# fnothaft/spark-bam

Hardware: AMD Instinct MI355X
Metric: compressed BAM GB/s for compute-splits + full-check (whole node, 1/2/4/8 GPU) (higher is better)
Workload: dtype u8

## Files before the change

spark-bam_amd/csrc/sbam_inflate.hip:

```cpp
#include <type_traits>

#include "sbam_internal.h"

namespace sbam {

#define SB_DEV __device__ __forceinline__

enum : int32_t { INF_OK = 0, INF_SHORT = 1, INF_DATA = 2, INF_OVERFLOW = 3 };

constexpr uint32_t kTokPad = 0x7fffu;
constexpr uint32_t kTokDist = 0x8000u;

SB_DEV uint64_t tok_region(int64_t uoff, int64_t b) {
  return (((uint64_t)uoff + 15) & ~15ull) + 32ull * (uint64_t)b;
}
SB_DEV int32_t tok_region_cap(int32_t us) { return (us + 16) / 2; }
SB_DEV uint64_t tok_arena_need(int32_t us) { return ((uint64_t)(2 * us + 32) + 15) & ~15ull; }

constexpr int kDecThreads = 256;
constexpr int kRows = 80;
constexpr int kLitSorted = 0;
constexpr int kClTab = 0;
constexpr int kLensLitRow = 32;
constexpr int kLensDistRow = 68;
constexpr int kDistSorted = 288;
constexpr int kEpoch = 4;
constexpr int kParkMin = 16;

constexpr uint8_t kClOrder[19] = {16, 17, 18, 0, 8, 7, 9, 6, 10, 5, 11, 4, 12, 3, 13, 2, 14, 1, 15};

struct Slice {
  uint8_t *base;
  SB_DEV uint8_t *b(int i) const { return base + (i >> 2) * (kDecThreads * 4) + (i & 3); }
  SB_DEV uint32_t *w(int row) const { return reinterpret_cast<uint32_t *>(base + row * (kDecThreads * 4)); }
};

template <int B, int E, class F>
SB_DEV void sfor(F &&f) {
  if constexpr (B < E) {
    f(std::integral_constant<int, B>{});
    sfor<B + 1, E>(f);
  }
}

struct Canon {
  uint32_t lim[16];
  int32_t pk[16];
};

SB_DEV int canon_decode(const Canon &c, uint64_t bb, int &len, bool &valid, int &hist) {
  const uint32_t rev = __builtin_bitreverse32((uint32_t)bb) >> 17;
  int32_t p = c.pk[1];
  sfor<1, 15>([&](auto I) {
    constexpr int l = decltype(I)::value;
    p = rev >= c.lim[l] ? c.pk[l + 1] : p;
  });
  const int L = p & 31;
  valid = rev < c.lim[15];
  len = valid ? L : 1;
  hist = (p >> 5) & 511;
  return valid ? (int)(rev >> (15 - L)) + (p >> 14) : 0;
}

SB_DEV int canon_decode_sel(const Canon &a, const Canon &b, bool useB, uint64_t bb, int &len, bool &valid,
                            int &hist) {
  const uint32_t rev = __builtin_bitreverse32((uint32_t)bb) >> 17;
  int32_t p = useB ? b.pk[1] : a.pk[1];
  sfor<1, 15>([&](auto I) {
    constexpr int l = decltype(I)::value;
    const uint32_t lim = useB ? b.lim[l] : a.lim[l];
    const int32_t pn = useB ? b.pk[l + 1] : a.pk[l + 1];
    p = rev >= lim ? pn : p;
  });
  const int L = p & 31;
  valid = rev < (useB ? b.lim[15] : a.lim[15]);
  len = valid ? L : 1;
  hist = (p >> 5) & 511;
  return valid ? (int)(rev >> (15 - L)) + (p >> 14) : 0;
}

struct Cnt15 {
  uint64_t a = 0, b = 0, c = 0;
  SB_DEV void add(uint32_t l, uint64_t v) {
    const uint32_t w = (l >= 7) + (l >= 14);
    const uint64_t inc = v << (9 * (l - 7 * w));
    a += w == 0 ? inc : 0ull;
    b += w == 1 ? inc : 0ull;
    c += w == 2 ? inc : 0ull;
  }
  SB_DEV uint32_t get(uint32_t l) const {
    const uint32_t w = (l >= 7) + (l >= 14);
    const uint64_t x = w == 0 ? a : w == 1 ? b : c;
    return (uint32_t)(x >> (9 * (l - 7 * w))) & 511u;
  }
};

template <int NW>
SB_DEV int canon_build(const uint32_t (&lens)[NW], const Slice &sl, int sorted_off, bool lit, Canon &c) {
  Cnt15 cnt, lo;
#pragma unroll
  for (int dw = 0; dw < NW; dw++) {
    const uint32_t w = lens[dw];
#pragma unroll 1
    for (int j = 0; j < 8; j++) {
      const uint32_t v = (w >> (4 * j)) & 15u;
      if (v) {
        cnt.add(v, 1);
        if (lit && dw * 8 + j < 256) lo.add(v, 1);
      }
    }
  }
  int left = 1, maxl = 0;
  bool over = false;
  uint32_t code = 0;
  int32_t offs = 0;
  Cnt15 cur;
  sfor<1, 16>([&](auto I) {
    constexpr int l = decltype(I)::value;
    const uint32_t k = cnt.get(l);
    left = 2 * left - (int)k;
    over |= left < 0;
    maxl = k ? l : maxl;
    c.lim[l] = (code + k) << (15 - l);
    const int32_t bse = offs - (int32_t)code;
    const uint32_t hist = (uint32_t)offs + (lit ? lo.get(l) : 0u);
    c.pk[l] = (int32_t)(((uint32_t)bse << 14) | (hist << 5) | (uint32_t)l);
    cur.add(l, (uint64_t)offs);
    offs += (int32_t)k;
    code = (code + k) << 1;
  });
  c.lim[0] = 0;
  c.pk[0] = 0;
  if (over || (left > 0 && maxl > 1)) return -1;
#pragma unroll
  for (int dw = 0; dw < NW; dw++) {
    const uint32_t w = lens[dw];
#pragma unroll 1
    for (int j = 0; j < 8; j++) {
      const uint32_t v = (w >> (4 * j)) & 15u;
      if (v) {
        const uint32_t pos = cur.get(v);
        cur.add(v, 1);
        *sl.b(sorted_off + (int)pos) = (uint8_t)(dw * 8 + j);
      }
    }
  }
  return 0;
}

SB_DEV uint32_t csel(uint64_t m, uint32_t a, uint32_t b) {
  uint32_t r;
  asm("v_cndmask_b32 %0, %1, %2, %3" : "=v"(r) : "v"(a), "v"(b), "s"(m));
  return r;
}
SB_DEV uint32_t sel16(const uint32_t (&A)[16], uint32_t i) {
  const uint64_t m0 = __builtin_amdgcn_ballot_w64((i & 1u) != 0), m1 = __builtin_amdgcn_ballot_w64((i & 2u) != 0),
                 m2 = __builtin_amdgcn_ballot_w64((i & 4u) != 0), m3 = __builtin_amdgcn_ballot_w64((i & 8u) != 0);
  uint32_t t[8], u[4];
#pragma unroll
  for (int k = 0; k < 8; k++) t[k] = csel(m0, A[2 * k], A[2 * k + 1]);
#pragma unroll
  for (int k = 0; k < 4; k++) u[k] = csel(m1, t[2 * k], t[2 * k + 1]);
  return csel(m3, csel(m2, u[0], u[1]), csel(m2, u[2], u[3]));
}

struct TokOut {
  uint32_t t0, t1, t2, t3;
  uint32_t p0, p1, p2, p3;
  int n;
  bool pend;
  uint64_t cur;
};

SB_DEV bool tok_store(TokOut &to, uint32_t a, uint32_t b, uint32_t c, uint32_t d, uint8_t *pool) {
  *reinterpret_cast<uint4 *>(pool + to.cur) = make_uint4(a, b, c, d);
  to.cur += 16;
  return true;
}

SB_DEV bool tok_put(TokOut &to, uint32_t t, uint8_t *pool) {
  to.t0 = __builtin_amdgcn_alignbit(to.t1, to.t0, 16);
  to.t1 = __builtin_amdgcn_alignbit(to.t2, to.t1, 16);
  to.t2 = __builtin_amdgcn_alignbit(to.t3, to.t2, 16);
  to.t3 = __builtin_amdgcn_alignbit(t, to.t3, 16);
  if (++to.n < 8) return true;
  bool ok = true;
  if (to.pend) ok = tok_store(to, to.p0, to.p1, to.p2, to.p3, pool);
  to.p0 = to.t0;
  to.p1 = to.t1;
  to.p2 = to.t2;
  to.p3 = to.t3;
  to.pend = true;
  to.n = 0;
  return ok;
}

enum : int { S_NEXT = 0, S_HDR = 1, S_HUFF = 2, S_STORED = 3, S_DONE = 4, S_EXIT = 5, S_PARK = 6 };


struct Bits {
  uint64_t bb;
  int bc;
  int left;
  uint32_t rp, nx;
  SB_DEV uint32_t peek(int n) const { return (uint32_t)bb & ((1u << n) - 1u); }
  SB_DEV void drop(int n) {
    bb >>= n;
    bc -= n;
    left -= n;
  }
  SB_DEV void refill_hbm(const uint32_t *src) {
    if (bc <= 32) {
      bb |= (uint64_t)src[rp] << bc;
      bc += 32;
      rp++;
    }
  }
};

__global__ __launch_bounds__(kDecThreads, 2) void k_inflate_slow(const uint8_t *__restrict__ d, int64_t D,
                                                                 BlockTable bt, TokPool tp,
                                                                 const int32_t *__restrict__ slow,
                                                                 const unsigned int *nslow,
                                                                 int32_t *__restrict__ status,
                                                                 int32_t *__restrict__ found,
                                                                 unsigned int *next_block) {
  __shared__ __attribute__((aligned(16))) uint8_t s_dec[kRows * kDecThreads * 4];
  const Slice sl{s_dec + 4 * threadIdx.x};
  const uint32_t *d32 = reinterpret_cast<const uint32_t *>(d);
  uint8_t *pool = tp.arena;

  int state = S_NEXT;
  int64_t blk = -1;
  const uint32_t *src = d32;
  uint32_t ldw = 0;
  Bits br{0, 0, 0, 0, 0};
  uint32_t A[16], B[8];
  uint32_t ws = 0;
#pragma unroll
  for (int k = 0; k < 16; k++) A[k] = 0;
#pragma unroll
  for (int k = 0; k < 8; k++) B[k] = 0;
  TokOut to{0, 0, 0, 0, 0, 0, 0, 0, 0, false, 0};
  Canon lc, dc;
  int32_t o = 0, us = 0, err = INF_OK, sleft = 0, fin = 0;
  bool drain = false;
  auto refill = [&]() {
    if (br.bc <= 32) {
      br.bb |= (uint64_t)br.nx << br.bc;
      br.bc += 32;
      br.rp++;
      br.nx = sel16(A, br.rp - ws);
    }
  };

  for (int it = 0;; it++) {
    if (state == S_NEXT) {
      const uint32_t i = atomicAdd(next_block, 1u);
      if (i >= *nslow) {
        state = S_EXIT;
      } else {
        blk = slow[i];
        const int64_t st = bt.start[blk];
        const int32_t hs = bt.hsize[blk], cs = bt.csize[blk];
        us = bt.usize[blk];
        o = 0;
        fin = 0;
        err = INF_OK;
        drain = false;
        const int32_t dlen = cs - hs - 8;
        if (us == 0) {
          state = S_DONE;
        } else if (us < 0 || us > 65536 || dlen < 0 || st + hs + dlen > D) {
          err = INF_DATA;
          state = S_DONE;
        } else {
          const uint64_t need = tok_arena_need(us);
          const uint64_t at = atomicAdd(tp.arena_used, (unsigned long long)need);
          if ((int64_t)(at + need) > tp.arena_cap) {
            err = INF_OVERFLOW;
            state = S_DONE;
          } else {
            tp.base[blk] = (int64_t)at;
            to.cur = at;
            to.n = 0;
            to.pend = false;
            const int64_t a = st + hs;
            src = d32 + (a >> 2);
            ldw = (uint32_t)(((a & 3) + dlen + 8 + 3) >> 2);
            const int skip = (int)(a & 3) * 8;
            br.bb = (uint64_t)src[0] >> skip;
            br.bc = 32 - skip;
            br.rp = 1;
            br.left = 8 * dlen;
            state = S_PARK;
          }
        }
      }
    }
    if ((it & (kEpoch - 1)) == 0) {
      if (__all(state == S_EXIT)) break;
      const uint64_t pk = __ballot(state == S_PARK);
      const uint64_t dc = __ballot(state == S_HUFF || state == S_STORED);
      if (pk && (__popcll(pk) >= kParkMin || dc == 0) && state == S_PARK) state = S_HDR;
    }
// ... 967 lines not shown
          tokA += cnt ? 1u : 0u;
          bytA += (cl ? lenv : 0u) + ((cnt && kind == K_LIT) ? 1u : 0u);
          pl = cl ? lenv : pl;
          st4 = live ? (cl ? 4u : 0u) : st4;
        };
        sfor<0, kCp>([&](auto J) {
          constexpr int jj = decltype(J)::value;
          const bool live = go && rp < seg_end;
          cp[jj] = (live && st4 == 0) ? (uint32_t)rp : ~0u;
          cc[jj] = tokA | (bytA << 12);
          if (__ballot(live) != 0) {
            if constexpr (jj * kCpSteps < kTR) {
              sfor<0, kCpSteps>([&](auto K) {
                constexpr int sj = jj * kCpSteps + decltype(K)::value;
                step(std::integral_constant<int, (sj < kTR ? sj : -1)>{});
              });
            } else {
#pragma unroll 2
              for (int k = 0; k < kCpSteps; k++) step(std::integral_constant<int, -1>{});
            }
          }
          if constexpr ((jj + 1) * kCpSteps == kTR) {
            stR = ((uint32_t)rp << 10) | (st4 << 7) | pl;
            bytR = bytA;
          }
        });
        while (__ballot(go && rp < seg_end) != 0) step(std::integral_constant<int, -1>{});
        exitEnd = ((uint32_t)rp << 10) | (st4 << 7) | pl;
      }
      WMARK(3);
      const SegResult own = nst > 0 ? SegResult{s1c & 4095u, s1c >> 12, s1e & ~1023u, (int)(s1e & 3u), false}
                                    : SegResult{tokA, bytA, exitEnd, ST_NONE, false};
      SegResult res = own;
      uint32_t nxt = lane == 0 ? own.exit : exitEnd;
      uint32_t bst = lane == 0 ? S : entry;
      bool ver = lane == 0;
      enum : int { kModeA = 0, kModeR = 1, kModeF = 2 };
      int mode = kModeA;
      uint32_t rjP = 0, rjs = 0, rjtk = 0;
      int f = 64;
      for (;;) {
        uint32_t pex = __shfl_up(nxt, 1);
        if (lane == 0) pex = S;
        bool upd = false;
        if (!ver && pex == bst) {
          ver = true;
          upd = nxt != own.exit;
          nxt = own.exit;
          res = own;
          mode = kModeA;
        }
        const uint64_t vs = __ballot(ver && res.stop != ST_NONE);
        f = uni(vs ? __ffsll((unsigned long long)vs) - 1 : 64);
        const bool need = lane > 0 && lane <= f && pex != bst;
        if (__ballot(need || upd) == 0) break;
        WADD(7, 1);
        if (need) {
          uint32_t st4 = (pex >> 7) & 4u;
          uint32_t pl = pex & 511u, tk = 0, by = 0;
          int rp = (int)(pex >> 10);
          auto next_cp = [&](uint32_t p) {
            uint32_t m = ~0u;
            sfor<0, kCp>([&](auto I) {
              const uint32_t x = cp[decltype(I)::value];
              m = (x >= p && x < m) ? x : m;
            });
            return m;
          };
          uint32_t tcp = next_cp((uint32_t)rp);
          mode = kModeF;
          for (;;) {
            if (st4 == 0 && (uint32_t)rp == tcp) {
              uint32_t cj = 0, sj = 0;
              sfor<0, kCp>([&](auto I) {
                const bool hit = cp[decltype(I)::value] == tcp;
                cj = hit ? cc[decltype(I)::value] : cj;
                sj = hit ? (uint32_t)(decltype(I)::value * kCpSteps) : sj;
              });
              const uint32_t P = tcp;
              mode = kModeR;
              rjP = P;
              rjs = sj;
              rjtk = tk;
              const bool h1 = nst >= 1 && s1p >= P, h2 = !h1 && nst >= 2 && s2p >= P;
              if (h1 || h2) {
                const uint32_t se = h1 ? s1e : s2e, sc = h1 ? s1c : s2c;
                res = SegResult{tk + (sc & 4095u) - (cj & 4095u), by + (sc >> 12) - (cj >> 12), se & ~1023u,
                                (int)(se & 3u), false};
                break;
              }
              if (nst <= 2) {
                res = SegResult{tk + tokA - (cj & 4095u), by + bytA - (cj >> 12), exitEnd, ST_NONE, false};
                break;
              }
              tcp = ~0u;
              mode = kModeF;
            }
            if (rp >= seg_end) {
              res = SegResult{tk, by, ((uint32_t)rp << 10) | (st4 << 7) | pl, ST_NONE, false};
              break;
            }
            uint32_t v;
            const uint32_t kind = wsym(wp, L, rp, st4, v);
            const bool outp = rp > pend;
            if (kind == K_SPEC || outp) {
              res = SegResult{tk, by, (uint32_t)rp << 10, outp ? ST_OUT : v == 0 ? ST_EOB : ST_ERR, false};
              break;
            }
            tk++;
            by += kind == K_LIT ? 1u : kind == K_LEN ? v - 253u : 0u;
            pl = kind == K_LEN ? v - 253u : pl;
            st4 = kind == K_LEN ? 4u : 0u;
            if ((uint32_t)rp > tcp) tcp = next_cp((uint32_t)rp);
          }
          nxt = res.stop != ST_NONE ? res.exit : res.exit;
          ver = true;
          bst = pex;
        }
      }
      WMARK(4);
      const bool act = lane <= f;
#ifdef SBAM_WAVE_STATS
      {
        const bool viaB = act && mode != kModeA;
        WADD(23, __ballot(act && mode == kModeF) != 0 ? 1 : 0);
        WADD(14, __popcll(__ballot(act)));
        WADD(15, __popcll(__ballot(viaB)));
        WADD(16, __popcll(__ballot(act && res.tok > 64)));
        WADD(17, __popcll(__ballot(act && res.tok > 96)));
        WADD(18, __popcll(__ballot(act && res.tok > 128)));
        WADD(19, __ballot(viaB) != 0 ? 1 : 0);
        WADD(20, __ballot(act && res.tok > 96) != 0 ? 1 : 0);
        WADD(21, __ballot(act && res.tok > 64) != 0 ? 1 : 0);
        WADD(22, __ballot(act && own.stop != ST_NONE) != 0 ? 1 : 0);
      }
#endif
      const uint32_t my_tok = act ? res.tok : 0u, my_byt = act ? res.byt : 0u;
      const uint32_t itok = wave_incl_scan(my_tok), ibyt = wave_incl_scan(my_byt);
      const uint32_t tot_tok = uni((uint32_t)__shfl(itok, 63)), tot_byt = uni((uint32_t)__shfl(ibyt, 63));
      const int stop_f = f < 64 ? uni(__shfl(res.stop, f)) : ST_NONE;
      if (stop_f == ST_ERR || stop_f == ST_OUT || out + (int)tot_byt > us || __ballot(act && res.bad) != 0) {
        ok = false;
        break;
      }
      if (ntok + (int)tot_tok > tcap) {
        const uint64_t need = tok_arena_need(us);
        uint64_t at = 0;
        if (lane == 0) at = atomicAdd(tp.arena_used, (unsigned long long)need);
        at = ((uint64_t)uni((uint32_t)__shfl((int)(at >> 32), 0)) << 32) | uni((uint32_t)__shfl((int)(uint32_t)at, 0));
        if ((int64_t)(at + need) > tp.arena_cap) {
          ok = false;
          break;
        }
        uint8_t *nreg = tp.arena + at;
        __builtin_amdgcn_fence(__ATOMIC_SEQ_CST, "workgroup");
        const int nb = 2 * ntok, nb16 = nb & ~15;
        for (int i = 16 * lane; i < nb16; i += 1024)
          *reinterpret_cast<uint4 *>(nreg + i) = *reinterpret_cast<const uint4 *>(reg + i);
        if (lane < (nb - nb16) / 2)
          reinterpret_cast<uint16_t *>(nreg + nb16)[lane] = reinterpret_cast<const uint16_t *>(reg + nb16)[lane];
        if (lane == 0) tp.base[b] = (int64_t)at;
        reg = nreg;
        tcap = 1 << 30;
      }
      bool tail = false;
      uint32_t tail_ti = 0, tail_st = 0;
      uint32_t r_lo = 0, r_hi = 0, r_tb = 0;
      if (act) {
        uint32_t start = __shfl_up(nxt, 1);
        if (lane == 0) start = S;
        uint32_t ti = (uint32_t)ntok + (itok - my_tok);
        auto run = [&](uint32_t st, int endp) {
          uint32_t st4 = (st >> 7) & 4u;
          int rp = (int)(st >> 10);
          while (rp < endp) {
            uint32_t v;
            const uint32_t kind = wsym(wp, L, rp, st4, v);
            if (kind == K_SPEC) break;
            st4 = kind == K_LEN ? 4u : 0u;
            *reinterpret_cast<uint16_t *>(reg + 2 * ti) = (uint16_t)v;
            ti++;
          }
        };
        WMARK(24);
        run(start, mode == kModeF ? seg_end : mode == kModeR ? (int)rjP : 0);
        WMARK(25);
        const uint32_t lo = mode == kModeR ? rjs : 0u;
        const uint32_t n = mode == kModeA ? res.tok : mode == kModeR ? res.tok - rjtk : 0u;
        const uint32_t hi = mode == kModeF ? 0u : min(lo + n, (uint32_t)kTR);
        const uint32_t tb = ti - lo;
        r_lo = lo;
        r_hi = hi;
        r_tb = tb;
        static_assert(kTR == 80, "one asm operand per register token dword");
        asm volatile("" : "+v"(tr[0]), "+v"(tr[1]), "+v"(tr[2]), "+v"(tr[3]), "+v"(tr[4]), "+v"(tr[5]), "+v"(tr[6]), "+v"(tr[7]), "+v"(tr[8]), "+v"(tr[9]), "+v"(tr[10]), "+v"(tr[11]), "+v"(tr[12]), "+v"(tr[13]), "+v"(tr[14]), "+v"(tr[15]), "+v"(tr[16]), "+v"(tr[17]), "+v"(tr[18]), "+v"(tr[19]), "+v"(tr[20]), "+v"(tr[21]), "+v"(tr[22]), "+v"(tr[23]), "+v"(tr[24]), "+v"(tr[25]), "+v"(tr[26]), "+v"(tr[27]), "+v"(tr[28]), "+v"(tr[29]), "+v"(tr[30]), "+v"(tr[31]), "+v"(tr[32]), "+v"(tr[33]), "+v"(tr[34]), "+v"(tr[35]), "+v"(tr[36]), "+v"(tr[37]), "+v"(tr[38]), "+v"(tr[39]));
        {
          const uint32_t par = tb & 1u;
          uint8_t *pa = reg + 2 * ((int64_t)ti - (int64_t)lo);
          if (par && lo == 0 && hi > 0) *reinterpret_cast<uint16_t *>(pa) = (uint16_t)tr[0];
          u32x4a *pv = reinterpret_cast<u32x4a *>(pa + 2 * par);
          uint32_t *pw = reinterpret_cast<uint32_t *>(pa + 2 * par);
          auto dw = [&](auto Q) {
            constexpr int q = decltype(Q)::value;
            const uint32_t nx = q + 1 < kTR / 2 ? tr[q + 1 < kTR / 2 ? q + 1 : q] : 0u;
            return par ? __builtin_amdgcn_alignbit(nx, tr[q], 16) : tr[q];
          };
          sfor<0, kTR / 8>([&](auto C) {
            constexpr int c = decltype(C)::value;
            const uint32_t a0 = dw(std::integral_constant<int, 4 * c>{}), a1 = dw(std::integral_constant<int, 4 * c + 1>{});
            const uint32_t a2 = dw(std::integral_constant<int, 4 * c + 2>{}), a3 = dw(std::integral_constant<int, 4 * c + 3>{});
            const uint32_t t0 = par + 8 * c;
            if (t0 >= lo && t0 + 8 <= hi) {
              pv[c] = u32x4a{a0, a1, a2, a3};
            } else if (t0 + 8 > lo && t0 < hi) {
              const uint32_t a[4] = {a0, a1, a2, a3};
#pragma unroll
              for (int k = 0; k < 4; k++) {
                const uint32_t u0 = t0 + 2 * k;
                const bool in0 = u0 >= lo && u0 < hi, in1 = u0 + 1 >= lo && u0 + 1 < hi;
                uint16_t *ph = reinterpret_cast<uint16_t *>(pw + 4 * c + k);
                if (in0 && in1) pw[4 * c + k] = a[k];
                else if (in0) ph[0] = (uint16_t)a[k];
                else if (in1) ph[1] = (uint16_t)(a[k] >> 16);
              }
            }
          });
        }
        WMARK(26);
        WMARK(27);
        tail = mode != kModeF && lo + n > (uint32_t)kTR;
        tail_st = lo <= (uint32_t)kTR ? stR : rjP << 10;
        tail_ti = lo <= (uint32_t)kTR ? tb + kTR : ti;
      }
      if (tail) {
        uint32_t st4 = (tail_st >> 7) & 4u, ti = tail_ti;
        int rp = (int)(tail_st >> 10);
        while (rp < seg_end) {
          uint32_t v;
          const uint32_t kind = wsym(wp, L, rp, st4, v);
          if (kind == K_SPEC) break;
          st4 = kind == K_LEN ? 4u : 0u;
          *reinterpret_cast<uint16_t *>(reg + 2 * ti) = (uint16_t)v;
          ti++;
        }
      }
      (void)r_lo;
      (void)r_hi;
      (void)r_tb;
      WMARK(28);
      out += (int)tot_byt;
      ntok += (int)tot_tok;
      if (f < 64) {
        pos = (int)(uni((uint32_t)__shfl(res.exit, f)) >> 10);
        break;
      }
      S = uni((uint32_t)__shfl(nxt, 63));
    }
  }
  if (ok && out != us) ok = false;
#ifdef SBAM_WAVE_STATS
  ws_[8] = __builtin_amdgcn_s_memtime() - wt0_;
  if (lane == 0)
    for (int i = 0; i < 29; i++) atomicAdd(&g_wave_stats[i], (unsigned long long)ws_[i]);
#endif
  if (lane == 0) {
    if (ok) {
      status[b] = INF_OK;
      found[b] = us;
    } else if (stored) {
      slow[bt.n + atomicAdd(nslow + 3, 1u)] = (int32_t)b;
    } else {
      slow[atomicAdd(nslow, 1u)] = (int32_t)b;
    }
  }
}

__global__ __launch_bounds__(64) void k_inflate_stored(const uint8_t *__restrict__ d, BlockTable bt, TokPool tp,
                                                      uint8_t *__restrict__ out, int32_t *__restrict__ status,
                                                      int32_t *__restrict__ found, int32_t *__restrict__ slow,
                                                      unsigned int *nslow) {
  __shared__ uint32_t seg[2 * kMaxStored];
  const unsigned n = nslow[3];
  for (unsigned i = blockIdx.x; i < n; i += gridDim.x) {
    const int64_t b = slow[bt.n + i];
    const int64_t a = bt.start[b] + bt.hsize[b], U0 = bt.uoff[b];
    const int32_t dlen = bt.csize[b] - bt.hsize[b] - 8, us = bt.usize[b];
    if (stored_copy(d, a, dlen, 0, us, out + U0, U0, seg)) {
      if (threadIdx.x == 0) {
        tp.base[b] = kTokDone;
        status[b] = INF_OK;
        found[b] = us;
      }
    } else if (threadIdx.x == 0) {
      slow[atomicAdd(nslow, 1u)] = (int32_t)b;
    }
    __syncthreads();
  }
}

namespace rs {
constexpr int kSpan = 1024;
constexpr int kFlush = 1024;
}

template <int RB>
struct RingGeom {
  static constexpr uint32_t kRing = 1u << RB, kMask = kRing - 1u, kDw = kRing / 4u, kDwMask = kDw - 1u;
  static constexpr uint32_t kMirror = 8u;
  static constexpr int kNear = (int)kRing - rs::kSpan - 264;
  static_assert(kNear >= rs::kSpan + rs::kFlush + 272, "far sources are in HBM");
  static_assert((int)kRing > rs::kSpan + 260 + rs::kFlush, "slots are flushed before reuse");
};

template <class G>
SB_DEV void ring_or1(uint32_t *ring, uint32_t i, uint32_t w) {
  atomicOr(ring + i, w);
  if (i < G::kMirror) atomicOr(ring + G::kDw + i, w);
}
template <class G>
SB_DEV void ring_or5(uint32_t *ring, uint32_t q, uint32_t w0, uint32_t w1, uint32_t w2, uint32_t w3, uint32_t w4) {
  if (q >= G::kMirror && q + 4u < G::kDw) {
    uint32_t *p = ring + q;
    atomicOr(p + 0, w0);
    atomicOr(p + 1, w1);
    atomicOr(p + 2, w2);
    atomicOr(p + 3, w3);
    atomicOr(p + 4, w4);
  } else {
    ring_or1<G>(ring, q & G::kDwMask, w0);
    ring_or1<G>(ring, (q + 1u) & G::kDwMask, w1);
    ring_or1<G>(ring, (q + 2u) & G::kDwMask, w2);
    ring_or1<G>(ring, (q + 3u) & G::kDwMask, w3);
    ring_or1<G>(ring, (q + 4u) & G::kDwMask, w4);
  }
}

template <int RB>
__global__ __launch_bounds__(64) void k_inflate_resolve(BlockTable bt, uint8_t *__restrict__ out, TokPool pool,
                                                        const int32_t *__restrict__ found,
                                                        const int32_t *__restrict__ list, int32_t *__restrict__ redo,
                                                        unsigned int *__restrict__ nredo) {
  using G = RingGeom<RB>;
  __shared__ __attribute__((aligned(16))) uint32_t ring[G::kDw + G::kMirror];
  __shared__ __attribute__((aligned(16))) uint32_t s_keep[17 * 4];
  uint8_t *ring8 = reinterpret_cast<uint8_t *>(ring);
  const int lane = (int)threadIdx.x;
  for (int i = lane; i < 17 * 4; i += 64) {
    const int n = i >> 2, k = i & 3, nb = n - 4 * k;
    s_keep[i] = nb >= 4 ? ~0u : nb <= 0 ? 0u : (1u << (8 * nb)) - 1u;
  }
  const int64_t b = list ? list[blockIdx.x] : blockIdx.x;
  const int ae = found[b];
  const int64_t tbase = pool.base[b];
  if (ae <= 0 || tbase == kTokDone) return;
  const int64_t U0 = bt.uoff[b];
  uint8_t *ob = out + U0;
  const uint32_t Gr = (uint32_t)U0 & G::kMask;
  const uint16_t *tk =
      reinterpret_cast<const uint16_t *>(tbase >= 0 ? pool.arena + tbase : pool.main + tok_region(U0, b));
  const int F0 = (int)((16 - (U0 & 15)) & 15);
  int F = F0;
  bool head = F0 == 0;
  int Z = -(int)(Gr & 3u);
  int B = 0, tp = 0;
  bool toofar = false;
  uint32_t ta = tk[2 * lane], tb = tk[2 * lane + 1], tn = tk[2 * lane + 2];
  asm volatile("" : "+v"(ta), "+v"(tb), "+v"(tn));
#ifdef SBAM_WAVE_STATS
  uint64_t rs_[8] = {0};
  uint32_t it_ = 0;
  uint64_t itw_ = 0, itl_ = 0;
  uint64_t rt_ = __builtin_amdgcn_s_memtime();
  const uint64_t rt0_ = rt_;
#endif
  while (B < ae) {
    const bool aLit = ta < 256u, aLen = (ta >> 8) == 1u, bLit = tb < 256u, bLen = (tb >> 8) == 1u;
    const int nl = (int)aLit + (int)bLit;
    const int Lm = aLen ? (int)ta - 253 : bLen ? (int)tb - 253 : 0;
    const int d = (int)((aLen ? tb : tn) & 0x7fffu) + 1;
    const int Ln = nl + Lm;
    const int incl = (int)wave_incl_scan((uint32_t)Ln);
    const int ex = incl - Ln;
    const int O = B + ex;
    const bool take = ex < rs::kSpan && O < ae;
    const uint64_t tmask = __ballot(take);
    const int nt = __popcll(tmask);
    const int E = min(B + __builtin_amdgcn_readlane(incl, nt - 1), ae);
    if (E <= B) break;
    const int tp2 = uni(tp + 2 * nt + (int)((__ballot(bLen) >> (nt - 1)) & 1ull));
    {
      const uint32_t z0 = (Gr + (uint32_t)Z) >> 2, z1 = (Gr + (uint32_t)E + 3u) >> 2;
#pragma unroll 1
      for (uint32_t k0 = z0; k0 < z1; k0 += 64u) {
        const uint32_t k = k0 + (uint32_t)lane, i = k & G::kDwMask;
        if (k < z1) {
          ring[i] = 0u;
          if (i < G::kMirror) ring[G::kDw + i] = 0u;
        }
      }
      Z = (int)(z1 * 4u - Gr);
    }
    RMARK(0);
    const int Ll = take ? min(nl, ae - O) : 0;
    if (Ll > 0) {
      const uint32_t lv = aLit ? (ta | (bLit ? tb << 8 : 0u)) : tb;
      const uint32_t x = (Gr + (uint32_t)O) & G::kMask;
      ring8[x] = (uint8_t)lv;
      if (x < 4u * G::kMirror) ring8[G::kRing + x] = (uint8_t)lv;
      if (Ll >= 2) {
        const uint32_t x1 = (x + 1u) & G::kMask;
        ring8[x1] = (uint8_t)(lv >> 8);
        if (x1 < 4u * G::kMirror) ring8[G::kRing + x1] = (uint8_t)(lv >> 8);
      }
    }
    RMARK(1);
    if (!head && B >= F0) {
      if (lane < F0) ob[lane] = ring8[(Gr + (uint32_t)lane) & G::kMask];
      head = true;
    }
    while (B - F >= rs::kFlush) {
      const uint32_t x = (Gr + (uint32_t)(F + 16 * lane)) & G::kMask;
      *reinterpret_cast<uint4 *>(ob + F + 16 * lane) = *reinterpret_cast<const uint4 *>(ring8 + x);
      F += rs::kFlush;
    }
    RMARK(2);
    const int mO = O + (bLen ? nl : 0);
    int Le = (take && Lm > 0) ? min(Lm, ae - mO) : 0;
    const bool tf = Le > 0 && d > mO;
    toofar |= tf;
    Le = tf ? 0 : Le;
    const bool mt = Le > 0;
    const bool far = d > G::kNear;
    const int srcEnd = mO - d + min(Le, d);
    u32x4 pf0 = {0u, 0u, 0u, 0u}, pf1 = {0u, 0u, 0u, 0u};
    if (mt && far) {
      pf0 = __builtin_nontemporal_load(reinterpret_cast<const u32x4 *>(ob + mO - d));
      if (Le > 16) pf1 = __builtin_nontemporal_load(reinterpret_cast<const u32x4 *>(ob + mO - d + 16));
    }
    uint32_t w2, n2;
    __builtin_memcpy(&w2, tk + tp2 + 2 * lane, 4);
    n2 = tk[tp2 + 2 * lane + 2];
    RMARK(3);
    uint64_t pend = __ballot(mt);
    const uint64_t below = (1ull << lane) - 1ull;
    const int mEnd = mO + Le;
    while (pend) {
      const int f = __ffsll((unsigned long long)pend) - 1;
      const int fr = __builtin_amdgcn_readlane(mO, f);
      const uint64_t pb = pend & below;
      const int jn = pb ? 63 - __clzll((long long)pb) : lane;
      const int endj = __shfl(mEnd, jn);
      uint64_t ready = pend & __ballot(srcEnd <= fr || pb == 0 || endj <= mO - d);
      if ((ready >> lane) & 1ull) {
        int done = 0, deff = d;
        while (done < Le) {
#ifdef SBAM_WAVE_STATS
          it_++;
#endif
          const int n = min(min(Le - done, 16), deff);
          const int src = mO + done - deff;
          const uint4 km = *reinterpret_cast<const uint4 *>(s_keep + 4 * n);
          uint32_t v0, v1, v2, v3;
          if (far) {
            if (done >= 32) {
              const u32x4 x = __builtin_nontemporal_load(reinterpret_cast<const u32x4 *>(ob + src));
              v0 = x.x; v1 = x.y; v2 = x.z; v3 = x.w;
              asm volatile("" : "+v"(v0), "+v"(v1), "+v"(v2), "+v"(v3));
            } else {
              const u32x4 x = done == 0 ? pf0 : pf1;
              v0 = x.x; v1 = x.y; v2 = x.z; v3 = x.w;
              asm volatile("" : "+v"(v0), "+v"(v1), "+v"(v2), "+v"(v3));
            }
          } else {
            const uint32_t xs = (Gr + (uint32_t)src) & G::kMask, qs = xs >> 2, ss = xs & 3u;
            const uint32_t *p = ring + qs;
            const uint32_t s0 = p[0], s1 = p[1], s2 = p[2], s3 = p[3], s4 = p[4];
            v0 = __builtin_amdgcn_alignbyte(s1, s0, ss);
            v1 = __builtin_amdgcn_alignbyte(s2, s1, ss);
            v2 = __builtin_amdgcn_alignbyte(s3, s2, ss);
            v3 = __builtin_amdgcn_alignbyte(s4, s3, ss);
          }
          v0 &= km.x;
          v1 &= km.y;
          v2 &= km.z;
          v3 &= km.w;
          const uint32_t xd = (Gr + (uint32_t)(mO + done)) & G::kMask, qd = xd >> 2, s8 = (xd & 3u) * 8u;
          const uint64_t a01 = ((uint64_t)v1 << 32 | v0) << s8, a12 = ((uint64_t)v2 << 32 | v1) << s8,
                         a23 = ((uint64_t)v3 << 32 | v2) << s8, a34 = (uint64_t)v3 << s8;
          ring_or5<G>(ring, qd, (uint32_t)a01, (uint32_t)(a01 >> 32), (uint32_t)(a12 >> 32), (uint32_t)(a23 >> 32),
                      (uint32_t)(a34 >> 32));
          done += n;
          if (n == deff && deff < 16) deff *= 2;
        }
      }
      pend &= ~ready;
#ifdef SBAM_WAVE_STATS
      rs_[7]++;
      {
        uint32_t mx = it_, sm = it_;
        for (int o = 32; o >= 1; o >>= 1) {
          mx = max(mx, (uint32_t)__shfl_xor((int)mx, o));
          sm += (uint32_t)__shfl_xor((int)sm, o);
        }
        itw_ += mx;
        itl_ += sm;
        it_ = 0;
      }
#endif
    }
    RMARK(4);
    B = E;
    asm volatile("" : "+v"(w2), "+v"(n2));
    ta = w2 & 0xffffu;
    tb = w2 >> 16;
    tn = n2;
    RMARK(5);
#ifdef SBAM_WAVE_STATS
    rs_[6]++;
#endif
    tp = tp2;
  }
  if (!head) {
    if (lane < min(F0, ae)) ob[lane] = ring8[(Gr + (uint32_t)lane) & G::kMask];
  }
  if (ae > F0) {
    const int Ft = F + ((ae - F) & ~15);
    for (int p = F + 16 * lane; p < Ft; p += rs::kFlush)
      *reinterpret_cast<uint4 *>(ob + p) = *reinterpret_cast<const uint4 *>(ring8 + ((Gr + (uint32_t)p) & G::kMask));
    if (Ft + lane < ae) ob[Ft + lane] = ring8[(Gr + (uint32_t)(Ft + lane)) & G::kMask];
  }
  if (__ballot(toofar) != 0 && lane == 0 && redo) redo[atomicAdd(nredo, 1u)] = (int32_t)b;
#ifdef SBAM_WAVE_STATS
  const uint64_t tot_ = __builtin_amdgcn_s_memtime() - rt0_;
  if (lane == 0) {
    for (int i = 0; i < 6; i++) atomicAdd(&g_wave_stats[32 + i], (unsigned long long)rs_[i]);
    atomicAdd(&g_wave_stats[38], (unsigned long long)rs_[6]);
    atomicAdd(&g_wave_stats[39], (unsigned long long)rs_[7]);
    atomicAdd(&g_wave_stats[31], (unsigned long long)tot_);
    atomicAdd(&g_wave_stats[29], (unsigned long long)itw_);
    atomicAdd(&g_wave_stats[30], (unsigned long long)itl_);
  }
#endif
}

__global__ void k_first_error(const int32_t *__restrict__ status, int64_t n, unsigned long long *first_err) {
  const int64_t i = (int64_t)blockIdx.x * blockDim.x + threadIdx.x;
  if (i < n && status[i] != INF_OK) atomicMin(first_err, (unsigned long long)i);
}

hipError_t launch_first_error(const int32_t *status, int64_t n, unsigned long long *first_err, hipStream_t s) {
  if (n == 0) return hipSuccess;
  hipLaunchKernelGGL(k_first_error, dim3((unsigned)((n + 255) / 256)), dim3(256), 0, s, status, n, first_err);
  return hipGetLastError();
}


hipError_t launch_inflate_decode(const uint8_t *d, int64_t D, BlockTable bt, TokPool tok, uint8_t *out,
                                 int32_t *status, int32_t *found, int32_t *slow, unsigned int *counters,
                                 hipStream_t s) {
  (void)hipMemsetAsync(counters, 0, 4 * sizeof(unsigned int), s);
  if (bt.n == 0) return hipSuccess;
  hipLaunchKernelGGL(k_inflate_wave, dim3((unsigned)bt.n), dim3(64), 0, s, d, D, bt, tok, status, found, slow,
                     counters + 0);
  hipLaunchKernelGGL(k_inflate_stored, dim3(4096), dim3(64), 0, s, d, bt, tok, out, status, found, slow,
                     counters + 0);
  hipLaunchKernelGGL(k_inflate_slow, dim3(256), dim3(kDecThreads), 0, s, d, D, bt, tok, slow, counters + 0, status,
                     found, counters + 1);
  return hipGetLastError();
}

hipError_t launch_inflate_resolve(BlockTable bt, uint8_t *out, TokPool tok, const int32_t *found,
                                  const int32_t *list, int64_t nlist, int32_t *redo, unsigned int *nredo,
                                  hipStream_t s) {
  const int64_t n = list ? nlist : bt.n;
  if (n == 0) return hipSuccess;
  hipLaunchKernelGGL(k_inflate_resolve<12>, dim3((unsigned)n), dim3(64), 0, s, bt, out, tok, found, list, redo, nredo);
  return hipGetLastError();
}

hipError_t launch_inflate_redo(const uint8_t *d, int64_t D, BlockTable bt, TokPool tok, const int32_t *list,
                               unsigned int *counters, int32_t *status, int32_t *found, hipStream_t s) {
  (void)hipMemsetAsync(counters + 1, 0, sizeof(unsigned int), s);
  hipLaunchKernelGGL(k_inflate_slow, dim3(256), dim3(kDecThreads), 0, s, d, D, bt, tok, list, counters + 2, status,
                     found, counters + 1);
  return hipGetLastError();
}

}
```

Baseline: 86.68.

## Resolve dependent LZ77 matches by source collapsing instead of serialized wave rounds

Replaces the iterative ready-mask loop, which serialized matches whose sources overlap other lanes' pending outputs, with a two-class scheme. Independent matches (source entirely before the batch start) copy in parallel. Dependent matches are laid out byte-per-lane and each byte's source is resolved by sweeping backwards through earlier matches, using modular period offsets to collapse overlapping copies to an already-final source byte. This removes multi-round ballot serialization but adds a per-dependent-byte readlane sweep over all dependent matches and byte-granular ring writes.

Measured after the change: 88.71 (median of 6 runs). +2.3%, better.

```diff
diff --git a/spark-bam_amd/csrc/sbam_inflate.hip b/spark-bam_amd/csrc/sbam_inflate.hip
--- a/spark-bam_amd/csrc/sbam_inflate.hip
+++ b/spark-bam_amd/csrc/sbam_inflate.hip
@@ -1,6 +1,7 @@
 #include <type_traits>
 
 #include "sbam_internal.h"
+#include "sbam_resolve_core.h"
 
 namespace sbam {
 
@@ -1574,6 +1575,7 @@
 constexpr int kSpan = 1024;
 constexpr int kFlush = 1024;
 }
+namespace rc = sbam_resolve;
 
 template <int RB>
 struct RingGeom {
@@ -1713,82 +1715,121 @@
     __builtin_memcpy(&w2, tk + tp2 + 2 * lane, 4);
     n2 = tk[tp2 + 2 * lane + 2];
     RMARK(3);
-    uint64_t pend = __ballot(mt);
-    const uint64_t below = (1ull << lane) - 1ull;
-    const int mEnd = mO + Le;
-    while (pend) {
-      const int f = __ffsll((unsigned long long)pend) - 1;
-      const int fr = __builtin_amdgcn_readlane(mO, f);
-      const uint64_t pb = pend & below;
-      const int jn = pb ? 63 - __clzll((long long)pb) : lane;
-      const int endj = __shfl(mEnd, jn);
-      uint64_t ready = pend & __ballot(srcEnd <= fr || pb == 0 || endj <= mO - d);
-      if ((ready >> lane) & 1ull) {
-        int done = 0, deff = d;
-        while (done < Le) {
+    static_assert(G::kNear > rc::kMaxMatch, "a dependent's source is near");
+    const bool ind = mt && srcEnd <= B;
+    const uint64_t dm = __ballot(mt && !ind);
+    uint64_t rem = dm;
+    int cut = 0;
+    int dsrc = 0, ddst = -1;
+    auto lay_out = [&]() {
+      int s = -(1 << 30), o = -1;
+      int t = 0, c = cut;
+      cut = 0;
+      uint64_t m = rem;
+      do {
+        const int k = 63 - __clzll((long long)m);
+        const uint64_t bit = 1ull << k;
+        m &= ~bit;
+        const int mk = __builtin_amdgcn_readlane(mO, k), dk = __builtin_amdgcn_readlane(d, k),
+                  lk = __builtin_amdgcn_readlane(Le, k);
+        const int r = s - mk;
+        const bool hit = rc::hop_hits(s, mk, lk);
+        const int left = lk - c, n = min(left, 64 - t);
+        const int jj = lane - t + (left - n);
+        const bool act = (uint32_t)(lane - t) < (uint32_t)n;
+        int rf = r, jf = jj;
+        if (lk > dk) {
+          int dv = dk;
+          asm volatile("" : "+v"(dv));
+          rf = rc::period_offset(r, dv);
+          jf = rc::period_offset(jj, dv);
+        }
+        const int base = mk - dk;
+        s = act ? base + jf : hit ? base + rf : s;
+        o = act ? mk + jj : o;
+        if (n == left) rem &= ~bit;
+        else if (t < 64) cut = c + n;
+        t += n;
+        c = 0;
+      } while (m);
+      dsrc = s;
+      ddst = o;
+    };
+    if (rem) lay_out();
+    if (ind) {
+      int done = 0, deff = d;
+      while (done < Le) {
 #ifdef SBAM_WAVE_STATS
-          it_++;
+        it_++;
 #endif
-          const int n = min(min(Le - done, 16), deff);
-          const int src = mO + done - deff;
-          const uint4 km = *reinterpret_cast<const uint4 *>(s_keep + 4 * n);
-          uint32_t v0, v1, v2, v3;
-          if (far) {
-            if (done >= 32) {
-              const u32x4 x = __builtin_nontemporal_load(reinterpret_cast<const u32x4 *>(ob + src));
-              v0 = x.x; v1 = x.y; v2 = x.z; v3 = x.w;
-              asm volatile("" : "+v"(v0), "+v"(v1), "+v"(v2), "+v"(v3));
-            } else {
-              const u32x4 x = done == 0 ? pf0 : pf1;
-              v0 = x.x; v1 = x.y; v2 = x.z; v3 = x.w;
-              asm volatile("" : "+v"(v0), "+v"(v1), "+v"(v2), "+v"(v3));
-            }
+        const int n = min(min(Le - done, 16), deff);
+        const int src = mO + done - deff;
+        const uint4 km = *reinterpret_cast<const uint4 *>(s_keep + 4 * n);
+        uint32_t v0, v1, v2, v3;
+        if (far) {
+          if (done >= 32) {
+            const u32x4 x = __builtin_nontemporal_load(reinterpret_cast<const u32x4 *>(ob + src));
+            v0 = x.x; v1 = x.y; v2 = x.z; v3 = x.w;
+            asm volatile("" : "+v"(v0), "+v"(v1), "+v"(v2), "+v"(v3));
           } else {
-            const uint32_t xs = (Gr + (uint32_t)src) & G::kMask, qs = xs >> 2, ss = xs & 3u;
-            const uint32_t *p = ring + qs;
-            const uint32_t s0 = p[0], s1 = p[1], s2 = p[2], s3 = p[3], s4 = p[4];
-            v0 = __builtin_amdgcn_alignbyte(s1, s0, ss);
-            v1 = __builtin_amdgcn_alignbyte(s2, s1, ss);
-            v2 = __builtin_amdgcn_alignbyte(s3, s2, ss);
-            v3 = __builtin_amdgcn_alignbyte(s4, s3, ss);
+            const u32x4 x = done == 0 ? pf0 : pf1;
+            v0 = x.x; v1 = x.y; v2 = x.z; v3 = x.w;
+            asm volatile("" : "+v"(v0), "+v"(v1), "+v"(v2), "+v"(v3));
           }
-          v0 &= km.x;
-          v1 &= km.y;
-          v2 &= km.z;
-          v3 &= km.w;
-          const uint32_t xd = (Gr + (uint32_t)(mO + done)) & G::kMask, qd = xd >> 2, s8 = (xd & 3u) * 8u;
-          const uint64_t a01 = ((uint64_t)v1 << 32 | v0) << s8, a12 = ((uint64_t)v2 << 32 | v1) << s8,
-                         a23 = ((uint64_t)v3 << 32 | v2) << s8, a34 = (uint64_t)v3 << s8;
-          ring_or5<G>(ring, qd, (uint32_t)a01, (uint32_t)(a01 >> 32), (uint32_t)(a12 >> 32), (uint32_t)(a23 >> 32),
-                      (uint32_t)(a34 >> 32));
-          done += n;
-          if (n == deff && deff < 16) deff *= 2;
-        }
-      }
-      pend &= ~ready;
+        } else {
+          const uint32_t xs = (Gr + (uint32_t)src) & G::kMask, qs = xs >> 2, ss = xs & 3u;
+          const uint32_t *p = ring + qs;
+          const uint32_t s0 = p[0], s1 = p[1], s2 = p[2], s3 = p[3], s4 = p[4];
+          v0 = __builtin_amdgcn_alignbyte(s1, s0, ss);
+          v1 = __builtin_amdgcn_alignbyte(s2, s1, ss);
+          v2 = __builtin_amdgcn_alignbyte(s3, s2, ss);
+          v3 = __builtin_amdgcn_alignbyte(s4, s3, ss);
+        }
+        v0 &= km.x;
+        v1 &= km.y;
+        v2 &= km.z;
+        v3 &= km.w;
+        const uint32_t xd = (Gr + (uint32_t)(mO + done)) & G::kMask, qd = xd >> 2, s8 = (xd & 3u) * 8u;
+        const uint64_t a01 = ((uint64_t)v1 << 32 | v0) << s8, a12 = ((uint64_t)v2 << 32 | v1) << s8,
+                       a23 = ((uint64_t)v3 << 32 | v2) << s8, a34 = (uint64_t)v3 << s8;
+        ring_or5<G>(ring, qd, (uint32_t)a01, (uint32_t)(a01 >> 32), (uint32_t)(a12 >> 32), (uint32_t)(a23 >> 32),
+                    (uint32_t)(a34 >> 32));
+        done += n;
+        if (n == deff && deff < 16) deff *= 2;
+      }
+    }
 #ifdef SBAM_WAVE_STATS
-      rs_[7]++;
-      {
-        uint32_t mx = it_, sm = it_;
-        for (int o = 32; o >= 1; o >>= 1) {
-          mx = max(mx, (uint32_t)__shfl_xor((int)mx, o));
-          sm += (uint32_t)__shfl_xor((int)sm, o);
-        }
-        itw_ += mx;
-        itl_ += sm;
-        it_ = 0;
-      }
+    {
+      uint32_t mx = it_, sm = it_;
+      for (int o = 32; o >= 1; o >>= 1) {
+        mx = max(mx, (uint32_t)__shfl_xor((int)mx, o));
+        sm += (uint32_t)__shfl_xor((int)sm, o);
+      }
+      itw_ += mx;
+      itl_ += sm;
+      it_ = 0;
+    }
 #endif
-    }
     RMARK(4);
+    for (;;) {
+      if (ddst >= 0) {
+        const uint8_t v = ring8[(Gr + (uint32_t)dsrc) & G::kMask];
+        const uint32_t x = (Gr + (uint32_t)ddst) & G::kMask;
+        ring8[x] = v;
+        if (x < 4u * G::kMirror) ring8[G::kRing + x] = v;
+      }
+      if (!rem) break;
+      lay_out();
+    }
+    RMARK(5);
     B = E;
     asm volatile("" : "+v"(w2), "+v"(n2));
     ta = w2 & 0xffffu;
     tb = w2 >> 16;
     tn = n2;
-    RMARK(5);
+    RMARK(6);
 #ifdef SBAM_WAVE_STATS
-    rs_[6]++;
+    rs_[7]++;
 #endif
     tp = tp2;
   }
@@ -1805,9 +1846,7 @@
 #ifdef SBAM_WAVE_STATS
   const uint64_t tot_ = __builtin_amdgcn_s_memtime() - rt0_;
   if (lane == 0) {
-    for (int i = 0; i < 6; i++) atomicAdd(&g_wave_stats[32 + i], (unsigned long long)rs_[i]);
-    atomicAdd(&g_wave_stats[38], (unsigned long long)rs_[6]);
-    atomicAdd(&g_wave_stats[39], (unsigned long long)rs_[7]);
+    for (int i = 0; i < 8; i++) atomicAdd(&g_wave_stats[32 + i], (unsigned long long)rs_[i]);
     atomicAdd(&g_wave_stats[31], (unsigned long long)tot_);
     atomicAdd(&g_wave_stats[29], (unsigned long long)itw_);
     atomicAdd(&g_wave_stats[30], (unsigned long long)itl_);
diff --git a/spark-bam_amd/csrc/sbam_resolve_core.h b/spark-bam_amd/csrc/sbam_resolve_core.h
--- /dev/null
+++ b/spark-bam_amd/csrc/sbam_resolve_core.h
@@ -0,0 +1,30 @@
+#pragma once
+#include <stdint.h>
+
+#if defined(__HIPCC__)
+#include <hip/hip_runtime.h>
+#define SBAM_RS_HD __host__ __device__ inline __attribute__((always_inline))
+#else
+#define SBAM_RS_HD inline
+#endif
+
+namespace sbam_resolve {
+
+constexpr int kMaxMatch = 258;
+
+SBAM_RS_HD int period_offset(int r, int d) { return r < d ? r : (int)((uint32_t)r % (uint32_t)d); }
+
+SBAM_RS_HD int collapsed_source(int mO, int d, int j) { return mO - d + period_offset(j, d); }
+
+SBAM_RS_HD bool hop_hits(int s, int mOk, int Lek) { return (uint32_t)(s - mOk) < (uint32_t)Lek; }
+
+SBAM_RS_HD int sweep_hop(int s, int mOk, int dk, int Lek) {
+  return hop_hits(s, mOk, Lek) ? collapsed_source(mOk, dk, s - mOk) : s;
+}
+
+SBAM_RS_HD int sweep(int s, const int *mO, const int *d, const int *Le, int n) {
+  for (int k = n - 1; k >= 0; k--) s = sweep_hop(s, mO[k], d[k], Le[k]);
+  return s;
+}
+
+}
```
